# XinMing0411/AC-VAE

Measured on AMD Instinct MI355X. Metric: train-step captions/s (and audio-sec/s) at B=32, 1/2/4/8 MI355X, higher is better.
Workload: dtype f32

## Files before the change

acvae_amd/csrc/decoder.hip:

```cpp
#include <cstdlib>
#include <vector>
#include "common.h"
#include "conv.h"
#include "rnn.h"
#include "decode_persist.h"
#include "text_common.h"

namespace {

inline int gemm2(const float* A1, long lda1, const float* B1, long ldb1, int K1, const float* A2, long lda2,
                 const float* B2, long ldb2, int K2, const float* bias, float* C, long ldc, int M, int N, int acc,
                 const Ctx& st) {
  if (M <= 64)
    return acvae_gemm_nt_dual(A1, lda1, B1, ldb1, K1, A2, lda2, B2, ldb2, K2, bias, C, ldc, M, N, acc, st.s, st.skws);
  ACVAE_TRY(acvae_gemm_nt_dual(A1, lda1, B1, ldb1, K1, nullptr, 0, nullptr, 0, 0, bias, C, ldc, M, N, acc, st.s, st.skws));
  return acvae_gemm_nt_dual(A2, lda2, B2, ldb2, K2, nullptr, 0, nullptr, 0, 0, nullptr, C, ldc, M, N, 1, st.s, st.skws);
}
struct TnWs { float* p; long bytes; };
inline int gemm_tn(const float* A, long lda, const float* B, long ldb, float* C, long ldc, int M, int N, int K, TnWs ws,
                   hipStream_t st) {
  return acvae_gemm_tn_fused(A, lda, B, ldb, C, ldc, M, N, K, 0, ws.p, ws.bytes, st);
}
struct TnBatch {
  TnGroup g;
// ... 825 lines not shown
  int64_t* words_c = (int64_t*)(sc + L.words_c);
  ACVAE_TRY(acvae::gather_words(words, Tc, 1, words_c, N, Tc, st));
  ACVAE_TRY(fork.begin());

  float* d_out = sc + L.d_out;
  if (d_outputs_ext) ACVAE_TRY(acvae::copy_rows(d_out, H, d_outputs_ext, H, R, H, st));
  else ACVAE_TRY(zero(d_out, (long)R * H, st));
  if (d_p_means_utt) {
    float* dhid = sc + L.dhid;
    ACVAE_TRY(gemm(d_p_means_utt, 2 * E, wt_mlo, 2 * E, nullptr, dhid, H, N, H, 2 * E, 0, st));
    ACVAE_TRY(acvae::pool_bwd(dhid, lens1, (const int*)(sv + L.pool_arg), d_out, (long)Tc * H, H, 1, N, Tc, H, st));
  }
  if (d_logits) ACVAE_TRY(gemm(d_logits, V, wt_cls, V, nullptr, d_out, H, R, H, V, 1, st));
  auto heads_params = [&](const Ctx& c, TnWs ws, double* dp) -> int {
    acvae::ColsumBatch cb;
    if (d_p_means_utt) {
      ACVAE_TRY(gemm_tn(d_p_means_utt, 2 * E, sv + L.pool_hid, H, G(TP_MLO_W), H, 2 * E, H, N, ws, c));
      cb.add({d_p_means_utt, N, 2 * E, G(TP_MLO_B)});
    } else if (G(TP_MLO_W) && G(TP_MLO_B)) {
      ACVAE_TRY(zero(G(TP_MLO_W), (long)2 * E * H, c));
      ACVAE_TRY(zero(G(TP_MLO_B), 2 * E, c));
    }
    if (d_logits) {
      ACVAE_TRY(gemm_tn(d_logits, V, outputs, H, G(TP_DEC_CLS_W), H, V, H, R, ws, c));
      cb.add({d_logits, R, V, G(TP_DEC_CLS_B)});
    } else {
      ACVAE_TRY(zero(G(TP_DEC_CLS_W), (long)V * H, c));
      ACVAE_TRY(zero(G(TP_DEC_CLS_B), V, c));
    }
    return acvae::colsum_batch(cb, dp, L.dpart_doubles, c);
  };
  static const bool heads_aux = !(getenv("ACVAE_HEADS_AUX") && atoi(getenv("ACVAE_HEADS_AUX")) == 0);
  const bool heads_on_aux = heads_aux && fork.on();
  if (heads_on_aux) {
    ACVAE_TRY(heads_params(sp, tn_p, dpart_p));
  } else if (!defer) {
    ACVAE_TRY(heads_params(st, tn, dpart));
  }

  float* dgi = sc + L.dgi;
  float* dgh = sc + L.dgh;
  float* dqd = sc + L.dqd;
  float* dencproj = sc + L.dencproj;
  float* dvpart = sc + L.dvpart;
  float* dctx = sc + L.dctx;
  float* dmem = sc + L.dmem;
  float* dh = sc + L.dh_a;
  float* dh2 = sc + L.dh_b;
  const float* gru_save = sv + L.gru_save;
  const float* hprev_d = sv + L.hprev_d;
  const float* qd = sv + L.qd;
  auto dec_begin = [&]() -> int {
    ACVAE_TRY(zero(dencproj, (long)N * S * A, st));
    ACVAE_TRY(zero(dvpart, (long)N * A, st));
    ACVAE_TRY(zero(dmem, (long)N * S * E, st));
    ACVAE_TRY(zero(dh, (long)N * H, st));
    return ACVAE_OK;
  };
  float* drnn = sc + L.drnn;
  float* dz_dec = sc + L.dz_dec;
  int dv_rows = N;
  auto dec_bptt = [&](int t) -> int {
    ACVAE_TRY(acvae::gru_bwd(dh, H, d_out + (long)t * H, (long)Tc * H, gru_save + (long)t * 4 * H, (long)Tc * 4 * H,
                             hprev_d + (long)t * H, (long)Tc * H, dgi + (long)t * 3 * H, (long)Tc * 3 * H,
                             dgh + (long)t * 3 * H, (long)Tc * 3 * H, dh2, H, nullptr, t, N, H, st));
    ACVAE_TRY(gemm(dgi + (long)t * 3 * H, (long)Tc * 3 * H, wt_dih + (long)E * 3 * H, 3 * H, nullptr, dctx, E, N, E,
                   3 * H, 0, st));
    ACVAE_TRY(acvae_attn_bwd(dctx, E, 0, qd + (long)t * A, (long)Tc * A, A, sv + L.encproj_d, mem, mem_lens,
                             P(TP_DEC_ATT_V), attn_w + (long)t * S, (long)Tc * S, S, dqd + (long)t * A, (long)Tc * A, A,
                             dencproj, dmem, dvpart, sc + L.attws, L.attws_bytes, N, 1, S, A, E, st));
    ACVAE_TRY(gemm2(dgh + (long)t * 3 * H, (long)Tc * 3 * H, wt_dhh, 3 * H, 3 * H, dqd + (long)t * A, (long)Tc * A,
                    wt_datt, A, A, nullptr, dh2, H, N, H, 1, st));
    float* tmp = dh; dh = dh2; dh2 = tmp;
    return ACVAE_OK;
  };
  auto dec_memgrad = [&]() -> int {
    return gemm(dencproj, A, wt_datt + (long)H * A, A, nullptr, dmem, E, N * S, E, A, 1, st);
  };
  auto dec_dz = [&](const Ctx& c) -> int {
    ACVAE_TRY(gemm(dgi, 3 * H, wt_dih + (long)2 * E * 3 * H, 3 * H, nullptr, dz_dec, E, R, E, 3 * H, 0, c));
    if (!d_q_z) return ACVAE_OK;
    if (!prior_feeds_decoder) {
      ACVAE_TRY(acvae::copy_rows(d_q_z, E, dz_dec, E, R, E, c));
    } else {
      for (int t = 0; t < Tc; ++t)
        ACVAE_TRY(acvae::copy_rows(d_q_z + (long)t * E, (long)Tc * E, dis_flags_host[t] ? nullptr : dz_dec + (long)t * E,
                                   (long)Tc * E, N, E, c));
    }
    return ACVAE_OK;
  };
  auto dec_tn = [&](TnBatch& tb) -> int {
    ACVAE_TRY(tb.add(dgi, 3 * H, rnn_d, 3 * E, G(TP_DEC_WIH), 3 * E, 3 * H, 3 * E, R));
    ACVAE_TRY(tb.add(dgh, 3 * H, hprev_d, H, G(TP_DEC_WHH), H, 3 * H, H, R));
    ACVAE_TRY(tb.add(dqd, A, hprev_d, H, G(TP_DEC_ATT_W), E + H, A, H, R));
    return tb.add(dencproj, A, mem, E, G(TP_DEC_ATT_W) + H, E + H, A, E, N * S);
  };
  auto dec_params = [&](const Ctx& c, TnWs ws, double* dp, bool with_dz = true, bool with_tn = true) -> int {
    if (with_tn) {
      TnBatch tb{{}, ws, c};
      ACVAE_TRY(dec_tn(tb));
      ACVAE_TRY(tb.launch());
    }
    {
      acvae::ColsumBatch cb;
      cb.add({dgi, R, 3 * H, G(TP_DEC_BIH)}); cb.add({dgh, R, 3 * H, G(TP_DEC_BHH)});
      cb.add({dencproj, N * S, A, G(TP_DEC_ATT_B)}); cb.add({dvpart, dv_rows, A, G(TP_DEC_ATT_V)});
      ACVAE_TRY(acvae::colsum_batch(cb, dp, L.dpart_doubles, c));
    }
    ACVAE_TRY(gemm(dgi, 3 * H, wt_dih, 3 * H, nullptr, drnn, E, R, E, 3 * H, 0, c));
    if (emb_keep)
      ACVAE_TRY(acvae::dropout_rows(drnn, (long)Tc * E, E, emb_keep, E, (long)N * E, emb_drop_p < 1.f ? 1.f / (1.f - emb_drop_p) : 0.f, N, Tc, E, c));
    if (with_dz) ACVAE_TRY(dec_dz(c));
// ... 52 lines not shown
  float* dqp = sc + L.dqp;
  auto prior_memgrad = [&]() -> int {
    ACVAE_TRY(gemm(dgates, 4 * Hp, wt_pih, 4 * Hp, nullptr, drnn_p, 3 * E, R, 2 * E, 4 * Hp, 0, sp));
    ACVAE_TRY(zero(dencproj_p, (long)N * S * E, sp));
    ACVAE_TRY(zero(dvpart_p, (long)N * E, sp));
    ACVAE_TRY(acvae_attn_bwd(drnn_p + E, (long)Tc * 3 * E, 3 * E, sv + L.qp, (long)Tc * E, E, sv + L.encproj_p, mem,
                             mem_lens, P(TP_P_ATT_V), sv + L.attw_p, (long)Tc * S, S, dqp, (long)Tc * E, E, dencproj_p,
                             dmem_p, dvpart_p, sc + L.attws_p, L.attws_bytes, N, Tc, S, E, E, sp));
    return gemm(dencproj_p, E, wt_patt + (long)E * E, E, nullptr, dmem_p, E, N * S, E, E, 1, sp);
  };
  auto prior_tn_bptt = [&](TnBatch& tb) -> int {
    ACVAE_TRY(tb.add(dgates, 4 * Hp, rnn_p, 3 * E, G(TP_P_WIH), 3 * E, 4 * Hp, 3 * E, R));
    ACVAE_TRY(tb.add(dgates, 4 * Hp, hpprev, Hp, G(TP_P_WHH), Hp, 4 * Hp, Hp, R));
    return tb.add(dml_all, 2 * E, hp_all, Hp, G(TP_P_ML_W), Hp, 2 * E, Hp, R);
  };
  auto prior_params = [&](bool with_bptt_tn = true) -> int {
    {
      TnBatch tb{{}, tn_p, sp};
      if (with_bptt_tn) ACVAE_TRY(prior_tn_bptt(tb));
      ACVAE_TRY(tb.add(dqp, E, rnn_p, 3 * E, G(TP_P_ATT_W), 2 * E, E, E, R));
      ACVAE_TRY(tb.add(dencproj_p, E, mem, E, G(TP_P_ATT_W) + E, 2 * E, E, E, N * S));
      ACVAE_TRY(tb.launch());
    }
    {
      acvae::ColsumBatch cb;
      cb.add({dml_all, R, 2 * E, G(TP_P_ML_B)}); cb.add({dgates, R, 4 * Hp, G(TP_P_BIH), G(TP_P_BHH)});
      cb.add({dencproj_p, N * S, E, G(TP_P_ATT_B)}); cb.add({dvpart_p, N, E, G(TP_P_ATT_V)});
      ACVAE_TRY(acvae::colsum_batch(cb, dpart_p, L.dpart_doubles, sp));
    }
    ACVAE_TRY(gemm(dqp, E, wt_patt, E, nullptr, drnn_p, 3 * E, R, E, E, 1, sp));
    return acvae::embed_scatter(words_c, drnn_p, 3 * E, G(TP_P_EMB), V, R, E, sp);
  };
  bool early_tn = false;
  if (prior_feeds_decoder) {
    ACVAE_TRY(dec_begin());
    for (int t = Tc - 1; t >= 0; --t) ACVAE_TRY(dec_bptt(t));
    ACVAE_TRY(dec_memgrad());
    ACVAE_TRY(dec_params(st, tn, dpart));
    if (fork.on()) ACVAE_TRY(Fork::edge(st.s, sp.s));
    ACVAE_TRY(prior_begin());
    for (int t = Tc - 1; t >= 0; --t) ACVAE_TRY(prior_bptt(t));
    ACVAE_TRY(prior_memgrad());
    ACVAE_TRY(prior_params());
  } else if (persist_bwd) {
    PbParams pb{};
    pb.wt_dhh = wt_dhh; pb.wt_datt = wt_datt; pb.wt_dih = wt_dih; pb.wt_phh = wt_phh; pb.wt_pih = wt_pih; pb.wt_pml = wt_pml;
    pb.att_v = P(TP_DEC_ATT_V);
    pb.encproj = sv + L.encproj_d; pb.mem = mem; pb.qd = qd; pb.attn_w = attn_w; pb.gru_save = gru_save; pb.hprev_d = hprev_d;
    pb.lstm_save = lstm_save; pb.c_all = c_all; pb.p_logs = p_logs; pb.eps_p = eps_p; pb.mem_lens = mem_lens;
    pb.d_out = d_out; pb.d_p_z = d_p_z; pb.d_p_means = d_p_means; pb.d_p_logs = d_p_logs;
    pb.dgi = dgi; pb.dgh = dgh; pb.dqd = dqd; pb.dctx = drnn;
    pb.dencproj = dencproj; pb.dmem = dmem; pb.dvpart = dvpart; pb.dgates = dgates; pb.dml_all = dml_all; pb.dhp = dhp;
    pb.dctx_part = sc + L.pd_part; pb.dhp_part = pb.dctx_part + 4L * N * E; pb.dml_part = pb.dhp_part + 4L * N * E;
    pb.cnt = (unsigned*)(sc + L.pd_cnt_b);
    pb.dqd_part = sc + L.pd_dqd; pb.ctx = rnn_d + E;
    pb.N = N; pb.Tc = Tc; pb.S = S; pb.E = E; pb.H = H; pb.A = A;
    ACVAE_TRY(acvae::decode_persist_bwd(pb, st.s, flags));
    dv_rows = N * acvae::decode_persist_bwd_rc_splits(S);
    ACVAE_TRY(dec_memgrad());
    if (fork.on()) ACVAE_TRY(Fork::edge(st.s, sp.s));
    ACVAE_TRY(prior_memgrad());
    if (!defer) {
      ACVAE_TRY(dec_params(st, tn, dpart));
      ACVAE_TRY(prior_params());
    } else {
      TnBatch tb{{}, tn, st.s};
      ACVAE_TRY(dec_tn(tb));
      ACVAE_TRY(prior_tn_bptt(tb));
      ACVAE_TRY(tb.launch());
      early_tn = true;
    }
  } else {
    ACVAE_TRY(dec_begin());
    ACVAE_TRY(prior_begin());
    for (int t = Tc - 1; t >= 0; --t) {
      ACVAE_TRY(dec_bptt(t));
      ACVAE_TRY(prior_bptt(t));
    }
    ACVAE_TRY(dec_memgrad());
    ACVAE_TRY(prior_memgrad());
    if (!defer) {
      ACVAE_TRY(dec_params(st, tn, dpart));
      ACVAE_TRY(prior_params());
    }
  }
  ACVAE_TRY(fork.join());
  ACVAE_TRY(acvae::add_rows(dmem, E, dmem_p, E, N * S, E, st));
  if (has_ln) {
    ACVAE_TRY(transp(P(TP_LN_W), Eenc, wt_ln, E, E, Eenc, st));
    ACVAE_TRY(gemm(dmem, E, wt_ln, E, nullptr, d_mem_in, Eenc, N * S, Eenc, E, 0, st));
    ACVAE_TRY(gemm_tn(dmem, E, mem_in, Eenc, G(TP_LN_W), Eenc, E, Eenc, N * S, tn, st));
    ACVAE_TRY(acvae::colsum2(dmem, N * S, E, dpart, G(TP_LN_B), nullptr, 0, st));
  } else {
    ACVAE_TRY(acvae::copy_rows(d_mem_in, E, dmem, E, N * S, E, st));
  }
  if (defer) {
    ACVAE_TRY(dec_dz(st));
    ACVAE_TRY(Fork::edge(st.s, sp.s));
    if (!heads_on_aux) ACVAE_TRY(heads_params(sp, tn_p, dpart_p));
    ACVAE_TRY(dec_params(sp, tn_p, dpart_p, false, !early_tn));
    ACVAE_TRY(prior_params(!early_tn));
  }
  return ACVAE_OK;
}

extern "C" int acvae_caps_to_long(const float* caps, int64_t* out, int64_t n, void* stream) {
  if (!caps || !out || n <= 0) return ACVAE_EINVAL;
  return acvae::caps_to_long(caps, out, (long)n, (hipStream_t)stream);
}
```

acvae_amd/csrc/gemm.hip:

```cpp
#include <cstdint>
#include <cstdlib>
#include "mfma_tile.h"
#include "../../include/acvae_hip.h"
#include "conv.h"

namespace {
using namespace mfma;

template <int BN, bool VEC4>
__global__ __launch_bounds__(nt_threads<128>(), 2) void gemm_nt_kernel(const float* __restrict__ A, long lda,
                                                                     const float* __restrict__ B, long ldb,
                                                                     const float* __restrict__ bias,
                                                                     float* __restrict__ C, long ldc, int M, int N,
                                                                     int K, int accumulate) {
  __shared__ NtSmem<128, BN> sm;
  PlainLoader<VEC4, 4> al{A, lda, M, K};
  PlainLoader<VEC4, BN / 32> bl{B, ldb, N, K};
  PlainEpilogue ep{C, ldc, bias, accumulate};
  int bm, bn;
  xcd_tile(gridDim.x, gridDim.y, bm, bn);
  nt_block<128, BN>(al, bl, M, N, K, bm, bn, ep, sm);
}

template <int WM, int WN, bool VEC4>
__global__ __launch_bounds__(256, 2) void gemm_tn_kernel(const float* __restrict__ A, long lda,
                                                         const float* __restrict__ B, long ldb, float* __restrict__ C,
                                                         long ldc, int M, int N, int K, int k_per, int accumulate,
                                                         long slab_stride) {
  __shared__ TnSmem<WM, WN> sm;
  PlainKMajorLoader<VEC4> al{A, lda, M, K}, bl{B, ldb, N, K};
  const int kb = blockIdx.z * k_per;
  const int ke = min(K, kb + k_per);
// ... 134 lines not shown
        b[u] = q0 + u < S ? __hip_atomic_load(reinterpret_cast<const unsigned long long*>(base + (long)(q0 + u) * 1024 + e),
                                              __ATOMIC_RELAXED, __HIP_MEMORY_SCOPE_AGENT) : 0ull;
#pragma unroll
      for (int u = 0; u < 8; ++u)
        if (q0 + u < S) { v0 += __uint_as_float((unsigned)b[u]); v1 += __uint_as_float((unsigned)(b[u] >> 32)); }
    }
    const int mm = e >> 5, m = m0 + mm;
#pragma unroll
    for (int k = 0; k < 2; ++k) {
      const int n = n0 + (e & 31) + k;
      if (m < M && n < N) {
        float v = k ? v1 : v0;
        if (bias) v += bias[n];
        float* p = C + (long)m * ldc + n;
        if (accumulate) v += *p;
        *p = v;
      }
    }
    return;
  }
  for (int e = threadIdx.x; e < 1024; e += SK_THREADS) {
    const int mm = e >> 5, nn = e & 31;
    const int m = m0 + mm, n = n0 + nn;
    if (m < M && n < N) {
      float v = 0.f;
#pragma unroll
      for (int w = 0; w < SK_WAVES; ++w) v += red[w][mm][nn];
      if (bias) v += bias[n];
      float* p = C + (long)m * ldc + n;
      if (accumulate) v += *p;
      *p = v;
    }
  }
}

__global__ void transpose_kernel(const float* __restrict__ in, long ld_in, float* __restrict__ out, long ld_out,
                                 int rows, int cols) {
  __shared__ float tile[32][33];
  const int c0 = blockIdx.x * 32, r0 = blockIdx.y * 32;
  for (int j = threadIdx.y; j < 32; j += 8) {
    const int r = r0 + j, c = c0 + threadIdx.x;
    tile[j][threadIdx.x] = (r < rows && c < cols) ? in[(long)r * ld_in + c] : 0.f;
  }
  __syncthreads();
  for (int j = threadIdx.y; j < 32; j += 8) {
    const int c = c0 + j, r = r0 + threadIdx.x;
    if (r < rows && c < cols) out[(long)c * ld_out + r] = tile[threadIdx.x][j];
  }
}

__global__ void transpose_batch_kernel(TransposeBatch b) {
  __shared__ float tile[32][33];
  const int m = b.find((int)blockIdx.x);
  const TransposeJob& job = b.job[m];
  const int t = blockIdx.x - b.start[m];
  const int tcols = (job.cols + 31) / 32;
  const int c0 = (t % tcols) * 32, r0 = (t / tcols) * 32;
  const float* in = job.in;
  float* out = job.out;
  const int rows = job.rows, cols = job.cols;
  for (int j = threadIdx.y; j < 32; j += 8) {
    const int r = r0 + j, c = c0 + threadIdx.x;
    tile[j][threadIdx.x] = (r < rows && c < cols) ? in[(long)r * job.ld_in + c] : 0.f;
  }
  __syncthreads();
  for (int j = threadIdx.y; j < 32; j += 8) {
// ... 66 lines not shown

int acvae_gemm_nt_pair(const float* A0, int64_t lda0, const float* B0, int64_t ldb0, int K0, const float* bias0, float* C0,
                       int64_t ldc0, int N0, int acc0, const float* A1, int64_t lda1, const float* B1, int64_t ldb1, int K1,
                       const float* bias1, float* C1, int64_t ldc1, int N1, int acc1, int M, hipStream_t st) {
  if (!A0 || !B0 || !C0 || !A1 || !B1 || !C1 || M <= 0 || M > 64 || N0 <= 0 || N1 <= 0 || K0 <= 0 || K1 <= 0)
    return ACVAE_EINVAL;
  const bool vec = vec_ok(A0, lda0, K0) && vec_ok(B0, ldb0, K0) && vec_ok(A1, lda1, K1) && vec_ok(B1, ldb1, K1);
  const SkProblem p0{A0, lda0, B0, ldb0, K0, bias0, C0, ldc0, N0, acc0}, p1{A1, lda1, B1, ldb1, K1, bias1, C1, ldc1, N1, acc1};
  const int nx0 = cdiv(N0, 32);
  dim3 grid(nx0 + cdiv(N1, 32), cdiv(M, 32));
  if (vec) hipLaunchKernelGGL(gemm_skinny_pair_kernel<true>, grid, dim3(SK_THREADS), 0, st, p0, p1, nx0, M);
  else hipLaunchKernelGGL(gemm_skinny_pair_kernel<false>, grid, dim3(SK_THREADS), 0, st, p0, p1, nx0, M);
  ACVAE_LAUNCH_CHECK();
  return ACVAE_OK;
}

static int skinny_plan(int M, int N, int Ktot, bool dual, bool have_ws) {
  const long big_blocks = (long)cdiv(M, 128) * cdiv(N, N <= 64 ? 64 : 128);
  if (!(M <= 64 || dual || (big_blocks < 100 && M <= 4096))) return 0;
  const int tiles = cdiv(N, 32) * cdiv(M, 32);
  int S = 1;
  static const bool splitk_on = !(getenv("ACVAE_SKINNY_SPLITK") && getenv("ACVAE_SKINNY_SPLITK")[0] == '0');
  if (have_ws && splitk_on && tiles <= 16 && Ktot >= 1024) {
    S = 128 / tiles;
    const int maxs = Ktot / 256;
    if (S > maxs) S = maxs;
    if (S > 8) S = 8;
    if (S < 1) S = 1;
    if ((long)tiles * S > SK_MAX_TILES) S = 1;
  }
  return S;
}

int acvae_gemm_nt_dual(const float* A1, int64_t lda1, const float* B1, int64_t ldb1, int K1, const float* A2,
                       int64_t lda2, const float* B2, int64_t ldb2, int K2, const float* bias, float* C, int64_t ldc,
                       int M, int N, int accumulate, hipStream_t st, float* skws) {
  if (!A1 || !B1 || !C || M <= 0 || N <= 0 || K1 <= 0) return ACVAE_EINVAL;
  if (A2 && (!B2 || K2 <= 0)) return ACVAE_EINVAL;
  bool vec = vec_ok(A1, lda1, K1) && vec_ok(B1, ldb1, K1);
  if (A2) vec = vec && vec_ok(A2, lda2, K2) && vec_ok(B2, ldb2, K2);
  const int S = skinny_plan(M, N, K1 + (A2 ? K2 : 0), A2 != nullptr, skws != nullptr);
  if (S > 0) {
    dim3 grid(cdiv(N, 32), cdiv(M, 32), S);
    unsigned* cnt = (unsigned*)skws;
    float* slabs = skws ? skws + SK_MAX_TILES : nullptr;
    if (vec)
      hipLaunchKernelGGL(gemm_skinny_kernel<true>, grid, dim3(SK_THREADS), 0, st, A1, lda1, B1, ldb1, K1, A2, lda2, B2,
                         ldb2, K2, bias, C, ldc, M, N, accumulate, slabs, cnt);
    else
      hipLaunchKernelGGL(gemm_skinny_kernel<false>, grid, dim3(SK_THREADS), 0, st, A1, lda1, B1, ldb1, K1, A2, lda2,
                         B2, ldb2, K2, bias, C, ldc, M, N, accumulate, slabs, cnt);
    ACVAE_LAUNCH_CHECK();
    return ACVAE_OK;
  }
  const bool bn64 = (N <= 64);
  dim3 grid(cdiv(M, 128), cdiv(N, bn64 ? 64 : 128));
#define LAUNCH_NT(BN_, V_)                                                                                     \
  hipLaunchKernelGGL((gemm_nt_kernel<BN_, V_>), grid, dim3(nt_threads<128>()), 0, st, A1, lda1, B1, ldb1, bias, C, ldc, M, \
                     N, K1, accumulate)
  if (bn64) { if (vec) LAUNCH_NT(64, true); else LAUNCH_NT(64, false); }
  else      { if (vec) LAUNCH_NT(128, true); else LAUNCH_NT(128, false); }
#undef LAUNCH_NT
  ACVAE_LAUNCH_CHECK();
  return ACVAE_OK;
}

extern "C" int acvae_gemm_nt(const float* A, int64_t lda, const float* B, int64_t ldb, const float* bias, float* C,
                             int64_t ldc, int M, int N, int K, int accumulate, void* stream) {
  return acvae_gemm_nt_dual(A, lda, B, ldb, K, nullptr, 0, nullptr, 0, 0, bias, C, ldc, M, N, accumulate,
                            (hipStream_t)stream, nullptr);
}

static int tn_splits(int M, int N, int K) {
  const long tiles = (long)cdiv(M, 128) * cdiv(N, 128);
  int s = (int)(256 / (tiles > 0 ? tiles : 1));
// ... 100 lines not shown
      tk += j.gx * j.gy;
    }
  }
  if (tk > TN_TICKETS) return -1;
  g.seal([](const TnJob& j) { return j.gx * j.gy * j.slices; });
  return slab;
}

int acvae_gemm_tn_group(TnGroup& g, float* ws, int64_t ws_bytes, hipStream_t st) {
  if (!g.ok()) return ACVAE_EINVAL;
  if (g.n <= 0) return ACVAE_OK;
  const long slab = acvae_gemm_tn_group_plan(g);
  if (slab < 0 || (slab > 0 && (!ws || ws_bytes < ((int64_t)TN_TICKETS + slab) * (int64_t)sizeof(float)))) return ACVAE_EWORKSPACE;
  hipLaunchKernelGGL(gemm_tn_group_kernel, dim3(g.start[g.n]), dim3(256), 0, st, g, ws + TN_TICKETS,
                     reinterpret_cast<unsigned*>(ws));
  ACVAE_LAUNCH_CHECK();
  return ACVAE_OK;
}

extern "C" int acvae_transpose(const float* in, int64_t ld_in, float* out, int64_t ld_out, int rows, int cols,
                               void* stream) {
  if (!in || !out || rows <= 0 || cols <= 0) return ACVAE_EINVAL;
  hipLaunchKernelGGL(transpose_kernel, dim3(cdiv(cols, 32), cdiv(rows, 32)), dim3(32, 8), 0, (hipStream_t)stream, in,
                     ld_in, out, ld_out, rows, cols);
  ACVAE_LAUNCH_CHECK();
  return ACVAE_OK;
}

extern "C" int64_t acvae_gemm_nt_splitk_workspace_bytes(void) { return acvae_skinny_ws_floats() * (int64_t)sizeof(float); }
extern "C" int acvae_gemm_nt_split_plan(int M, int N, int K1, int K2, int with_ws) {
  if (M <= 0 || N <= 0 || K1 <= 0 || K2 < 0) return ACVAE_EINVAL;
  return skinny_plan(M, N, K1 + K2, K2 > 0, with_ws != 0);
}
extern "C" int acvae_gemm_nt_dual_ws(const float* A1, int64_t lda1, const float* B1, int64_t ldb1, int K1, const float* A2,
                                     int64_t lda2, const float* B2, int64_t ldb2, int K2, const float* bias, float* C,
                                     int64_t ldc, int M, int N, int accumulate, float* ws, int64_t ws_bytes, int reset_tickets,
                                     void* stream) {
  if (!A1 || !B1 || !C || M <= 0 || N <= 0 || K1 <= 0 || (A2 && (!B2 || K2 <= 0))) return ACVAE_EINVAL;
  if (ws && ws_bytes < acvae_gemm_nt_splitk_workspace_bytes()) return ACVAE_EWORKSPACE;
  hipStream_t st = (hipStream_t)stream;
  if (ws && reset_tickets) ACVAE_TRY(acvae_skinny_ws_reset(ws, st));
  return acvae_gemm_nt_dual(A1, lda1, B1, ldb1, K1, A2, lda2, B2, ldb2, K2, bias, C, ldc, M, N, accumulate, st, ws);
}
extern "C" int acvae_gemm_nt_pair_c(const float* A0, int64_t lda0, const float* B0, int64_t ldb0, int K0, const float* bias0,
                                    float* C0, int64_t ldc0, int N0, int acc0, const float* A1, int64_t lda1, const float* B1,
                                    int64_t ldb1, int K1, const float* bias1, float* C1, int64_t ldc1, int N1, int acc1, int M,
                                    void* stream) {
  return acvae_gemm_nt_pair(A0, lda0, B0, ldb0, K0, bias0, C0, ldc0, N0, acc0, A1, lda1, B1, ldb1, K1, bias1, C1, ldc1, N1,
                            acc1, M, (hipStream_t)stream);
}
extern "C" int64_t acvae_gemm_tn_fused_workspace_bytes(int M, int N, int K) {
  if (M <= 0 || N <= 0 || K <= 0) return -1;
  const int s = tn_splits(M, N, K);
  return s > 1 ? (int64_t)TN_TICKETS * 4 + (int64_t)s * M * N * (int64_t)sizeof(float) : 0;
}
extern "C" int acvae_gemm_tn_fused_plan(int M, int N, int K, int64_t ws_bytes) {
  if (M <= 0 || N <= 0 || K <= 0) return ACVAE_EINVAL;
  return tn_fused_slices(M, N, K, ws_bytes > 0, ws_bytes, nullptr);
}
extern "C" int acvae_gemm_tn_fused_c(const float* A, int64_t lda, const float* B, int64_t ldb, float* C, int64_t ldc, int M,
                                     int N, int K, int accumulate, float* ws, int64_t ws_bytes, int reset_tickets,
                                     void* stream) {
  if (!A || !B || !C || M <= 0 || N <= 0 || K <= 0) return ACVAE_EINVAL;
  hipStream_t st = (hipStream_t)stream;
  if (ws && reset_tickets && ws_bytes >= (int64_t)TN_TICKETS * 4)
    if (hipMemsetAsync(ws, 0, TN_TICKETS * sizeof(unsigned), st) != hipSuccess) return (int)hipGetLastError();
// ... 34 lines not shown
```

acvae_amd/csrc/mfma_tile.h:

```cpp
#pragma once
#include <type_traits>
#include "common.h"

namespace mfma {

constexpr int BK = 32;
constexpr int LDS_LD = BK + 4;
constexpr int KT = BK / 4;
constexpr int NT_LOADERS = 256;
constexpr int RPP = NT_LOADERS / KT;

template <int BMT, int BN>
struct alignas(16) NtSmem {
  alignas(16) float a[2][BMT * LDS_LD];
  alignas(16) float b[2][BN * LDS_LD];
};
template <int BMT>
constexpr int nt_threads() { return (BMT / 32 + 4) * 64; }

__device__ __forceinline__ void xcd_tile(int nm, int nn, int& bm, int& bn) {
#ifdef ACVAE_NO_XCD_REMAP
  bm = blockIdx.x; bn = blockIdx.y; return;
#endif
  const int total = nm * nn;
// ... 343 lines not shown
  constexpr int SK_U = 8;
  int g = wave;
  for (; g < Gfull; g += SK_U * nwaves) {
    float4 a[SK_U], b[SK_U];
#pragma unroll
    for (int u = 0; u < SK_U; ++u) {
      const int gu = g + u * nwaves;
      const long off = (gu < Gfull) ? (long)gu * 8 : 0;
      a[u] = *reinterpret_cast<const float4*>(ap + off);
      b[u] = *reinterpret_cast<const float4*>(bp + off);
    }
#pragma unroll
    for (int u = 0; u < SK_U; ++u) {
      const bool ok = (g + u * nwaves) < Gfull;
      const float4 av = ok ? a[u] : make_float4(0.f, 0.f, 0.f, 0.f);
      acc = __builtin_amdgcn_mfma_f32_32x32x2f32(av.x, b[u].x, acc, 0, 0, 0);
      acc = __builtin_amdgcn_mfma_f32_32x32x2f32(av.y, b[u].y, acc, 0, 0, 0);
      acc = __builtin_amdgcn_mfma_f32_32x32x2f32(av.z, b[u].z, acc, 0, 0, 0);
      acc = __builtin_amdgcn_mfma_f32_32x32x2f32(av.w, b[u].w, acc, 0, 0, 0);
    }
  }
  g = Gfull + ((wave - Gfull % nwaves) % nwaves + nwaves) % nwaves;
  for (; g < G; g += nwaves) {
    const int k = g * 8 + 4 * lh;
    const float4 a = sk_load<VEC4>(ap - 4 * lh, k, K);
    const float4 b = sk_load<VEC4>(bp - 4 * lh, k, K);
    acc = __builtin_amdgcn_mfma_f32_32x32x2f32(a.x, b.x, acc, 0, 0, 0);
    acc = __builtin_amdgcn_mfma_f32_32x32x2f32(a.y, b.y, acc, 0, 0, 0);
    acc = __builtin_amdgcn_mfma_f32_32x32x2f32(a.z, b.z, acc, 0, 0, 0);
    acc = __builtin_amdgcn_mfma_f32_32x32x2f32(a.w, b.w, acc, 0, 0, 0);
  }
}

}
```

acvae_amd/csrc/rnn.h:

```cpp
#pragma once
#include <hip/hip_runtime.h>
#include <stdint.h>
#include "job_table.h"
namespace acvae {
int caps_to_long(const float* caps, int64_t* out, long n, hipStream_t st);
int select_word(const int64_t* caps, long ld_caps, const int64_t* seqs, long ld_seqs, int64_t* words, long ld_words,
                int t, int use_caps, int start_idx, int N, hipStream_t st);
int finish_rows(int64_t* seqs, long ld_seqs, uint8_t* unfinished, int t, int end_idx, int N, hipStream_t st);
int embed_gather(const int64_t* words, long w_stride, const float* table, int V, float* out, long ld_out, int rows,
                 int E, hipStream_t st);
int embed_scatter(const int64_t* words_contig, const float* d, long ld_d, float* dtable, int V, int rows, int E,
                  hipStream_t st);
int dropout_rows(float* x, long ld_n, long ld_t, const uint8_t* keep, long k_sn, long k_st, float scale, int N, int cnt,
                 int E, hipStream_t st);
int gather_words(const int64_t* src, long s_sn, long s_st, int64_t* dst, int N, int T, hipStream_t st);
int gru_fwd(const float* gi, long ld_gi, const float* gh, long ld_gh, const float* hp, long ld_hp, float* ho,
            long ld_ho, float* oseq, long ld_os, float* save, long ld_sv, float* hps, long ld_hps, const int64_t* lens,
            int t, int N, int H, hipStream_t st);
int gru_bwd(const float* dh_next, long ld_dn, const float* d_out, long ld_do, const float* save, long ld_sv,
            const float* hps, long ld_hps, float* dgi, long ld_dgi, float* dgh, long ld_dgh, float* dh_prev, long ld_dp,
            const int64_t* lens, int t, int N, int H, hipStream_t st);
int lstm_fwd(const float* gates, long ld_g, const float* cp, long ld_cp, float* ho, long ld_ho, float* co, long ld_co,
             float* save, long ld_sv, int N, int H, hipStream_t st);
int lstm_bwd(const float* dh, long ld_dh, const float* dc_next, long ld_dc, const float* save, long ld_sv,
             const float* cp, long ld_cp, float* dgates, long ld_dg, float* dc_prev, long ld_dcp, int N, int H,
             hipStream_t st);
int pool_fwd(const float* x, long ld_n, long ld_t, const int64_t* lens, float* out, int* argmax, int N, int T, int C,
             hipStream_t st);
int pool_bwd(const float* d, const int64_t* lens, const int* argmax, float* dx, long ld_n, long ld_t, int accumulate,
             int N, int T, int C, hipStream_t st);
int colsum_rows(const float* x, long ld, int rows, int cols, float* out, int accumulate, hipStream_t st);
int add_rows(float* dst, long ld_d, const float* src, long ld_s, int rows, int cols, hipStream_t st);
int copy_rows(float* dst, long ld_d, const float* src, long ld_s, int rows, int cols, hipStream_t st);
struct CopyRowsJob { float* dst; long ld_d; const float* src; long ld_s; int rows, cols; };
using CopyRowsBatch = JobTable<CopyRowsJob, 8>;
int copy_rows_batch(const CopyRowsBatch& b, hipStream_t st);
struct ZeroRegion { void* p; long words; };
struct ZeroBatch : JobTable<ZeroRegion, 16> {
  void add(void* p, long words) { if (p && words > 0) JobTable::add({p, words}); }
};
int zero_batch(const ZeroBatch& b, hipStream_t st);
}
```

acvae_amd/csrc/rnn.hip:

```cpp
#include "common.h"
#include "rnn.h"

namespace {

constexpr int TH = 256;
inline int grid1(long n) {
  long b = (n + TH - 1) / TH;
  return (int)(b < 1 ? 1 : (b > 4096 ? 4096 : b));
}

__global__ void caps_to_long_kernel(const float* __restrict__ caps, int64_t* __restrict__ out, long n) {
  for (long i = blockIdx.x * (long)TH + threadIdx.x; i < n; i += (long)gridDim.x * TH) out[i] = (int64_t)caps[i];
}
__global__ void select_word_kernel(const int64_t* __restrict__ caps, long ld_caps, const int64_t* __restrict__ seqs,
                                   long ld_seqs, int64_t* __restrict__ words, long ld_words, int t, int use_caps,
                                   int start_idx, int N) {
  const int n = blockIdx.x * TH + threadIdx.x;
  if (n >= N) return;
  int64_t w;
  if (use_caps) w = caps[n * ld_caps + t];
  else if (t == 0) w = start_idx;
  else w = seqs[n * ld_seqs + t - 1];
  words[n * ld_words + t] = w;
}
// ... 190 lines not shown
                                int accumulate, int N, int T, int C) {
  const long total = (long)N * T * C;
  for (long i = blockIdx.x * (long)TH + threadIdx.x; i < total; i += (long)gridDim.x * TH) {
    const int c = (int)(i % C);
    const int t = (int)((i / C) % T);
    const int n = (int)(i / ((long)C * T));
    const int len = (int)lens[n];
    float g = 0.f;
    if (t < len) {
      const float dv = d[n * C + c];
      g = dv / (float)len + (argmax[n * C + c] == t ? dv : 0.f);
    }
    float* p = dx + n * ld_n + t * ld_t + c;
    *p = accumulate ? *p + g : g;
  }
}

__global__ void colsum_rows_kernel(const float* __restrict__ x, long ld, int rows, int cols, float* __restrict__ out,
                                   int accumulate) {
  const int c = blockIdx.x * TH + threadIdx.x;
  if (c >= cols) return;
  float a = 0.f;
  for (int r = 0; r < rows; ++r) a += x[r * ld + c];
  out[c] = accumulate ? out[c] + a : a;
}
__global__ void add_rows_kernel(float* __restrict__ dst, long ld_d, const float* __restrict__ src, long ld_s, int rows,
                                int cols) {
  const long total = (long)rows * cols;
  for (long i = blockIdx.x * (long)TH + threadIdx.x; i < total; i += (long)gridDim.x * TH) {
    const int r = (int)(i / cols), c = (int)(i % cols);
    dst[r * ld_d + c] += src[r * ld_s + c];
  }
}
__global__ void copy_rows_kernel(float* __restrict__ dst, long ld_d, const float* __restrict__ src, long ld_s, int rows,
                                 int cols) {
  const long total = (long)rows * cols;
  for (long i = blockIdx.x * (long)TH + threadIdx.x; i < total; i += (long)gridDim.x * TH) {
    const int r = (int)(i / cols), c = (int)(i % cols);
    dst[r * ld_d + c] = src ? src[r * ld_s + c] : 0.f;
  }
}

__global__ void copy_rows_batch_kernel(acvae::CopyRowsBatch b) {
  const acvae::CopyRowsJob& j = b.job[blockIdx.y];
  const long total = (long)j.rows * j.cols;
  for (long i = blockIdx.x * (long)TH + threadIdx.x; i < total; i += (long)gridDim.x * TH) {
    const int r = (int)(i / j.cols), c = (int)(i % j.cols);
    j.dst[r * j.ld_d + c] = j.src ? j.src[r * j.ld_s + c] : 0.f;
  }
}

__global__ void zero_batch_kernel(acvae::ZeroBatch b) {
  unsigned* p = static_cast<unsigned*>(b.job[blockIdx.y].p);
  const long n = b.job[blockIdx.y].words;
  for (long i = blockIdx.x * (long)TH + threadIdx.x; i < n; i += (long)gridDim.x * TH) p[i] = 0u;
}

}

namespace acvae {
#define LAUNCH(k, g, ...) hipLaunchKernelGGL(k, dim3(g), dim3(TH), 0, st, __VA_ARGS__)
int zero_batch(const ZeroBatch& b, hipStream_t st) {
  if (!b.ok()) return ACVAE_EINVAL;
  if (b.n <= 0) return ACVAE_OK;
  long most = 1;
  for (int j = 0; j < b.n; ++j) if (b.job[j].words > most) most = b.job[j].words;
// ... 61 lines not shown
         ld_dgh, dh_prev, ld_dp, lens, t, N, H);
  ACVAE_LAUNCH_CHECK(); return ACVAE_OK;
}
int lstm_fwd(const float* gates, long ld_g, const float* cp, long ld_cp, float* ho, long ld_ho, float* co, long ld_co,
             float* save, long ld_sv, int N, int H, hipStream_t st) {
  LAUNCH(lstm_fwd_kernel, grid1((long)N * H), gates, ld_g, cp, ld_cp, ho, ld_ho, co, ld_co, save, ld_sv, N, H);
  ACVAE_LAUNCH_CHECK(); return ACVAE_OK;
}
int lstm_bwd(const float* dh, long ld_dh, const float* dc_next, long ld_dc, const float* save, long ld_sv,
             const float* cp, long ld_cp, float* dgates, long ld_dg, float* dc_prev, long ld_dcp, int N, int H,
             hipStream_t st) {
  LAUNCH(lstm_bwd_kernel, grid1((long)N * H), dh, ld_dh, dc_next, ld_dc, save, ld_sv, cp, ld_cp, dgates, ld_dg, dc_prev,
         ld_dcp, N, H);
  ACVAE_LAUNCH_CHECK(); return ACVAE_OK;
}
int pool_fwd(const float* x, long ld_n, long ld_t, const int64_t* lens, float* out, int* argmax, int N, int T, int C,
             hipStream_t st) {
  LAUNCH(pool_fwd_kernel, grid1((long)N * C), x, ld_n, ld_t, lens, out, argmax, N, T, C);
  ACVAE_LAUNCH_CHECK(); return ACVAE_OK;
}
int pool_bwd(const float* d, const int64_t* lens, const int* argmax, float* dx, long ld_n, long ld_t, int accumulate,
             int N, int T, int C, hipStream_t st) {
  LAUNCH(pool_bwd_kernel, grid1((long)N * T * C), d, lens, argmax, dx, ld_n, ld_t, accumulate, N, T, C);
  ACVAE_LAUNCH_CHECK(); return ACVAE_OK;
}
int colsum_rows(const float* x, long ld, int rows, int cols, float* out, int accumulate, hipStream_t st) {
  LAUNCH(colsum_rows_kernel, cdiv(cols, TH), x, ld, rows, cols, out, accumulate);
  ACVAE_LAUNCH_CHECK(); return ACVAE_OK;
}
int add_rows(float* dst, long ld_d, const float* src, long ld_s, int rows, int cols, hipStream_t st) {
  LAUNCH(add_rows_kernel, grid1((long)rows * cols), dst, ld_d, src, ld_s, rows, cols);
  ACVAE_LAUNCH_CHECK(); return ACVAE_OK;
}
int copy_rows(float* dst, long ld_d, const float* src, long ld_s, int rows, int cols, hipStream_t st) {
  LAUNCH(copy_rows_kernel, grid1((long)rows * cols), dst, ld_d, src, ld_s, rows, cols);
  ACVAE_LAUNCH_CHECK(); return ACVAE_OK;
}
#undef LAUNCH
}
```

include/acvae_hip.h:

```cpp
#ifndef ACVAE_HIP_H
#define ACVAE_HIP_H
#include <stdint.h>
#ifdef __cplusplus
extern "C" {
#endif

#define ACVAE_ABI_VERSION 3
int acvae_abi_version(void);

#define ACVAE_FLAG_NO_PERSIST 1
#define ACVAE_FLAG_DEFER_PARAM_GRADS 2
#define ACVAE_FLAG_NO_ATTN_SPLIT 4
#define ACVAE_FLAG_ROLLOUT_GRAD 16
#define ACVAE_FLAG_TEST_STALL 8

int acvae_persist_status_register(int device, void* status_words_host);

int acvae_gemm_nt(const float* A, int64_t lda, const float* B, int64_t ldb, const float* bias, float* C,
                  int64_t ldc, int M, int N, int K, int accumulate, void* stream);
int acvae_gemm_tn(const float* A, int64_t lda, const float* B, int64_t ldb, float* C, int64_t ldc, int M, int N,
                  int K, int accumulate, float* slab_ws, int64_t slab_ws_bytes, void* stream);
int64_t acvae_gemm_tn_workspace_bytes(int M, int N, int K);
int64_t acvae_colsum_workspace_bytes(int cols);
int acvae_colsum(const float* x, int rows, int cols, float* out, void* ws, int64_t ws_bytes, void* stream);

int64_t acvae_gemm_nt_splitk_workspace_bytes(void);
int acvae_gemm_nt_split_plan(int M, int N, int K1, int K2, int with_ws);
int acvae_gemm_nt_dual_ws(const float* A1, int64_t lda1, const float* B1, int64_t ldb1, int K1, const float* A2,
                          int64_t lda2, const float* B2, int64_t ldb2, int K2, const float* bias, float* C, int64_t ldc,
                          int M, int N, int accumulate, float* ws, int64_t ws_bytes, int reset_tickets, void* stream);
int acvae_gemm_nt_pair_c(const float* A0, int64_t lda0, const float* B0, int64_t ldb0, int K0, const float* bias0, float* C0,
                         int64_t ldc0, int N0, int acc0, const float* A1, int64_t lda1, const float* B1, int64_t ldb1, int K1,
                         const float* bias1, float* C1, int64_t ldc1, int N1, int acc1, int M, void* stream);
int64_t acvae_gemm_tn_fused_workspace_bytes(int M, int N, int K);
int acvae_gemm_tn_fused_plan(int M, int N, int K, int64_t ws_bytes);
int acvae_gemm_tn_fused_c(const float* A, int64_t lda, const float* B, int64_t ldb, float* C, int64_t ldc, int M, int N,
                          int K, int accumulate, float* ws, int64_t ws_bytes, int reset_tickets, void* stream);
int64_t acvae_gemm_tn_group_workspace_bytes(int n, const int* M, const int* N, const int* K);
int acvae_gemm_tn_group_c(int n, const void* const* A, const int64_t* lda, const void* const* B, const int64_t* ldb,
                          const void* const* C, const int64_t* ldc, const int* M, const int* N, const int* K, void* ws,
                          int64_t ws_bytes, int reset_tickets, void* stream);
int64_t acvae_colsum_batch_workspace_bytes(int n, const int* P, const int* width);
int acvae_colsum_batch_plan(int n, const int* P, const int* width, int64_t ws_bytes);
int acvae_colsum_batch(int n, const void* const* x, const int* P, const int* width, const void* const* out,
                       const void* const* out_b, void* ws, int64_t ws_bytes, int reset_tickets, void* stream);
int acvae_transpose(const float* in, int64_t ld_in, float* out, int64_t ld_out, int rows, int cols, void* stream);

int64_t acvae_attn_fwd_workspace_bytes(int N, int Tq, int S, int A, int E);
int acvae_attn_fwd(const float* qproj, int64_t q_sn, int64_t q_sj, const float* encproj, const float* enc,
                   const int64_t* lens, const float* v, float* ctx, int64_t c_sn, int64_t c_sj, float* weights,
                   int64_t w_sn, int64_t w_sj, int N, int Tq, int S, int A, int E, void* ws, int64_t ws_bytes, void* stream,
                   int flags);
int acvae_tanh_att(const float* x, float* y, int64_t n, void* stream);
int64_t acvae_attn_bwd_workspace_bytes(int N, int Tq, int S, int A);
int acvae_attn_bwd(const float* dctx, int64_t dc_sn, int64_t dc_sj, const float* qproj, int64_t q_sn, int64_t q_sj,
                   const float* encproj, const float* enc, const int64_t* lens, const float* v,
                   const float* weights, int64_t w_sn, int64_t w_sj, float* dqproj, int64_t dq_sn, int64_t dq_sj,
                   float* dencproj, float* denc, float* dv_part, float* ws, int64_t ws_bytes, int N, int Tq, int S,
                   int A, int E, void* stream);

// ... 277 lines not shown
```

Measured before the change: 2116.

## Add register-blocked skinny GEMM, fuse backward glue copies, reorder heads fork

Result: no change. 2131 (median of 6 runs) (+0.7%).

```diff
diff --git a/acvae_amd/csrc/decoder.hip b/acvae_amd/csrc/decoder.hip
--- a/acvae_amd/csrc/decoder.hip
+++ b/acvae_amd/csrc/decoder.hip
@@ -881,7 +881,9 @@
   };
   static const bool heads_aux = !(getenv("ACVAE_HEADS_AUX") && atoi(getenv("ACVAE_HEADS_AUX")) == 0);
   const bool heads_on_aux = heads_aux && fork.on();
+  static const bool sw_heads_late = !(getenv("ACVAE_HEADS_LATE") && atoi(getenv("ACVAE_HEADS_LATE")) == 0);
   if (heads_on_aux) {
+    if (sw_heads_late) ACVAE_TRY(Fork::edge(st.s, sp.s));
     ACVAE_TRY(heads_params(sp, tn_p, dpart_p));
   } else if (!defer) {
     ACVAE_TRY(heads_params(st, tn, dpart));
@@ -926,7 +928,10 @@
   auto dec_memgrad = [&]() -> int {
     return gemm(dencproj, A, wt_datt + (long)H * A, A, nullptr, dmem, E, N * S, E, A, 1, st);
   };
+  static const bool sw_glue = !(getenv("ACVAE_BWD_GLUE") && atoi(getenv("ACVAE_BWD_GLUE")) == 0);
   auto dec_dz = [&](const Ctx& c) -> int {
+    if (sw_glue && d_q_z && !prior_feeds_decoder)
+      return gemm(dgi, 3 * H, wt_dih + (long)2 * E * 3 * H, 3 * H, nullptr, d_q_z, E, R, E, 3 * H, 0, c);
     ACVAE_TRY(gemm(dgi, 3 * H, wt_dih + (long)2 * E * 3 * H, 3 * H, nullptr, dz_dec, E, R, E, 3 * H, 0, c));
     if (!d_q_z) return ACVAE_OK;
     if (!prior_feeds_decoder) {
@@ -1045,6 +1050,7 @@
     return acvae::embed_scatter(words_c, drnn_p, 3 * E, G(TP_P_EMB), V, R, E, sp);
   };
   bool early_tn = false;
+  bool early_dz = false;
   if (prior_feeds_decoder) {
     ACVAE_TRY(dec_begin());
     for (int t = Tc - 1; t >= 0; --t) ACVAE_TRY(dec_bptt(t));
@@ -1077,6 +1083,7 @@
       ACVAE_TRY(dec_params(st, tn, dpart));
       ACVAE_TRY(prior_params());
     } else {
+      if (sw_glue) { ACVAE_TRY(dec_dz(st)); early_dz = true; }
       TnBatch tb{{}, tn, st.s};
       ACVAE_TRY(dec_tn(tb));
       ACVAE_TRY(prior_tn_bptt(tb));
@@ -1098,17 +1105,19 @@
     }
   }
   ACVAE_TRY(fork.join());
-  ACVAE_TRY(acvae::add_rows(dmem, E, dmem_p, E, N * S, E, st));
+  if (has_ln || !sw_glue) ACVAE_TRY(acvae::add_rows(dmem, E, dmem_p, E, N * S, E, st));
   if (has_ln) {
     ACVAE_TRY(transp(P(TP_LN_W), Eenc, wt_ln, E, E, Eenc, st));
     ACVAE_TRY(gemm(dmem, E, wt_ln, E, nullptr, d_mem_in, Eenc, N * S, Eenc, E, 0, st));
     ACVAE_TRY(gemm_tn(dmem, E, mem_in, Eenc, G(TP_LN_W), Eenc, E, Eenc, N * S, tn, st));
     ACVAE_TRY(acvae::colsum2(dmem, N * S, E, dpart, G(TP_LN_B), nullptr, 0, st));
+  } else if (sw_glue) {
+    ACVAE_TRY(acvae::sum_rows(d_mem_in, E, dmem, E, dmem_p, E, N * S, E, st));
   } else {
     ACVAE_TRY(acvae::copy_rows(d_mem_in, E, dmem, E, N * S, E, st));
   }
   if (defer) {
-    ACVAE_TRY(dec_dz(st));
+    if (!early_dz) ACVAE_TRY(dec_dz(st));
     ACVAE_TRY(Fork::edge(st.s, sp.s));
     if (!heads_on_aux) ACVAE_TRY(heads_params(sp, tn_p, dpart_p));
     ACVAE_TRY(dec_params(sp, tn_p, dpart_p, false, !early_tn));
diff --git a/acvae_amd/csrc/gemm.hip b/acvae_amd/csrc/gemm.hip
--- a/acvae_amd/csrc/gemm.hip
+++ b/acvae_amd/csrc/gemm.hip
@@ -1,3 +1,4 @@
+#include <atomic>
 #include <cstdint>
 #include <cstdlib>
 #include "mfma_tile.h"
@@ -198,6 +199,47 @@
       *p = v;
     }
   }
+}
+
+template <int BM, int BN, int U>
+__global__ __launch_bounds__(SK_THREADS) void gemm_skinny_blocked_kernel(const float* __restrict__ A, long lda,
+                                                                         const float* __restrict__ B, long ldb, int K,
+                                                                         const float* __restrict__ bias,
+                                                                         float* __restrict__ C, long ldc, int M, int N,
+                                                                         int accumulate) {
+  __shared__ float red[SK_WAVES][32][33];
+  const int lane = threadIdx.x & 63, wave = threadIdx.x >> 6, li = lane & 31, lh = lane >> 5;
+  const int n0 = blockIdx.x * (32 * BN), m0 = blockIdx.y * (32 * BM);
+  f32x16 acc[BM][BN];
+#pragma unroll
+  for (int i = 0; i < BM; ++i)
+#pragma unroll
+    for (int j = 0; j < BN; ++j)
+#pragma unroll
+      for (int r = 0; r < 16; ++r) acc[i][j][r] = 0.f;
+  sk_accumulate_blocked<BM, BN, U>(acc, A, lda, B, ldb, M, N, K, m0, n0, wave, li, lh);
+#pragma unroll
+  for (int i = 0; i < BM; ++i)
+#pragma unroll
+    for (int j = 0; j < BN; ++j) {
+      if (i | j) __syncthreads();
+#pragma unroll
+      for (int r = 0; r < 16; ++r) red[wave][(r & 3) + 8 * (r >> 2) + 4 * lh][li] = acc[i][j][r];
+      __syncthreads();
+      for (int e = threadIdx.x; e < 1024; e += SK_THREADS) {
+        const int mm = e >> 5, nn = e & 31;
+        const int m = m0 + 32 * i + mm, n = n0 + 32 * j + nn;
+        if (m < M && n < N) {
+          float v = 0.f;
+#pragma unroll
+          for (int w = 0; w < SK_WAVES; ++w) v += red[w][mm][nn];
+          if (bias) v += bias[n];
+          float* p = C + (long)m * ldc + n;
+          if (accumulate) v += *p;
+          *p = v;
+        }
+      }
+    }
 }
 
 __global__ void transpose_kernel(const float* __restrict__ in, long ld_in, float* __restrict__ out, long ld_out,
@@ -330,6 +372,58 @@
   return S;
 }
 
+static int device_cus() {
+  static std::atomic<int> cached[64];
+  int dev = 0;
+  if (hipGetDevice(&dev) != hipSuccess || dev < 0 || dev >= 64) { (void)hipGetLastError(); return 256; }
+  int n = cached[dev].load(std::memory_order_relaxed);
+  if (n == 0) {
+    if (hipDeviceGetAttribute(&n, hipDeviceAttributeMultiprocessorCount, dev) != hipSuccess || n <= 0) {
+      (void)hipGetLastError();
+      n = 256;
+    }
+    cached[dev].store(n, std::memory_order_relaxed);
+  }
+  return n;
+}
+static int skinny_block(int M, int N, int S, bool dual) {
+  static const bool on = !(getenv("ACVAE_SK_BLOCK") && atoi(getenv("ACVAE_SK_BLOCK")) == 0);
+  if (S != 1 || dual || !on) return 11;
+  const int tm = cdiv(M, 32), tn = cdiv(N, 32);
+  if ((long)tm * tn < device_cus()) return 11;
+  if (N > M) return tn >= 2 ? 12 : 11;
+  return tm >= 2 ? 21 : 11;
+}
+
+constexpr int SK_BLOCK_U = 4;
+template <int BM, int BN>
+static void launch_blocked(const float* A, int64_t lda, const float* B, int64_t ldb, int K, const float* bias, float* C,
+                           int64_t ldc, int M, int N, int accumulate, hipStream_t st) {
+  dim3 grid(cdiv(N, 32 * BN), cdiv(M, 32 * BM));
+  hipLaunchKernelGGL((gemm_skinny_blocked_kernel<BM, BN, SK_BLOCK_U>), grid, dim3(SK_THREADS), 0, st, A, lda, B, ldb, K, bias,
+                     C, ldc, M, N, accumulate);
+}
+static int skinny_launch(int block, const float* A, int64_t lda, const float* B, int64_t ldb, int K, const float* bias,
+                         float* C, int64_t ldc, int M, int N, int accumulate, hipStream_t st) {
+  switch (block) {
+    case 21: launch_blocked<2, 1>(A, lda, B, ldb, K, bias, C, ldc, M, N, accumulate, st); break;
+    case 12: launch_blocked<1, 2>(A, lda, B, ldb, K, bias, C, ldc, M, N, accumulate, st); break;
+    case 11: {
+      dim3 grid(cdiv(N, 32), cdiv(M, 32), 1);
+      if (vec_ok(A, lda, K) && vec_ok(B, ldb, K))
+        hipLaunchKernelGGL(gemm_skinny_kernel<true>, grid, dim3(SK_THREADS), 0, st, A, lda, B, ldb, K, nullptr, 0, nullptr, 0,
+                           0, bias, C, ldc, M, N, accumulate, nullptr, nullptr);
+      else
+        hipLaunchKernelGGL(gemm_skinny_kernel<false>, grid, dim3(SK_THREADS), 0, st, A, lda, B, ldb, K, nullptr, 0, nullptr, 0,
+                           0, bias, C, ldc, M, N, accumulate, nullptr, nullptr);
+      break;
+    }
+    default: return ACVAE_EINVAL;
+  }
+  ACVAE_LAUNCH_CHECK();
+  return ACVAE_OK;
+}
+
 int acvae_gemm_nt_dual(const float* A1, int64_t lda1, const float* B1, int64_t ldb1, int K1, const float* A2,
                        int64_t lda2, const float* B2, int64_t ldb2, int K2, const float* bias, float* C, int64_t ldc,
                        int M, int N, int accumulate, hipStream_t st, float* skws) {
@@ -339,6 +433,8 @@
   if (A2) vec = vec && vec_ok(A2, lda2, K2) && vec_ok(B2, ldb2, K2);
   const int S = skinny_plan(M, N, K1 + (A2 ? K2 : 0), A2 != nullptr, skws != nullptr);
   if (S > 0) {
+    const int block = vec ? skinny_block(M, N, S, A2 != nullptr) : 11;
+    if (block != 11) return skinny_launch(block, A1, lda1, B1, ldb1, K1, bias, C, ldc, M, N, accumulate, st);
     dim3 grid(cdiv(N, 32), cdiv(M, 32), S);
     unsigned* cnt = (unsigned*)skws;
     float* slabs = skws ? skws + SK_MAX_TILES : nullptr;
@@ -505,6 +601,18 @@
   if (M <= 0 || N <= 0 || K1 <= 0 || K2 < 0) return ACVAE_EINVAL;
   return skinny_plan(M, N, K1 + K2, K2 > 0, with_ws != 0);
 }
+extern "C" int acvae_gemm_nt_block_plan(int M, int N, int K1, int K2, int with_ws) {
+  if (M <= 0 || N <= 0 || K1 <= 0 || K2 < 0) return ACVAE_EINVAL;
+  const int S = skinny_plan(M, N, K1 + K2, K2 > 0, with_ws != 0);
+  return S > 0 ? skinny_block(M, N, S, K2 > 0) : 0;
+}
+extern "C" int acvae_gemm_nt_blocked_c(const float* A, int64_t lda, const float* B, int64_t ldb, const float* bias, float* C,
+                                       int64_t ldc, int M, int N, int K, int accumulate, int bm, int bn, void* stream) {
+  if (!A || !B || !C || M <= 0 || N <= 0 || K <= 0 || lda < K || ldb < K || ldc < N) return ACVAE_EINVAL;
+  if (bm < 1 || bn < 1 || bm * bn > 2) return ACVAE_EINVAL;
+  if (bm * bn > 1 && !(vec_ok(A, lda, K) && vec_ok(B, ldb, K))) return ACVAE_EALIGN;
+  return skinny_launch(bm * 10 + bn, A, lda, B, ldb, K, bias, C, ldc, M, N, accumulate, (hipStream_t)stream);
+}
 extern "C" int acvae_gemm_nt_dual_ws(const float* A1, int64_t lda1, const float* B1, int64_t ldb1, int K1, const float* A2,
                                      int64_t lda2, const float* B2, int64_t ldb2, int K2, const float* bias, float* C,
                                      int64_t ldc, int M, int N, int accumulate, float* ws, int64_t ws_bytes, int reset_tickets,
diff --git a/acvae_amd/csrc/mfma_tile.h b/acvae_amd/csrc/mfma_tile.h
--- a/acvae_amd/csrc/mfma_tile.h
+++ b/acvae_amd/csrc/mfma_tile.h
@@ -399,4 +399,54 @@
   }
 }
 
-}
+template <int BM, int BN, int U>
+__device__ __forceinline__ void sk_accumulate_blocked(f32x16 (&acc)[BM][BN], const float* A, long lda, const float* B,
+                                                      long ldb, int M, int N, int K, int m0, int n0, int wave, int li,
+                                                      int lh) {
+  const float* ap[BM];
+  const float* bp[BN];
+#pragma unroll
+  for (int i = 0; i < BM; ++i) ap[i] = A + (long)((m0 + 32 * i + li) < M ? m0 + 32 * i + li : 0) * lda + 4 * lh;
+#pragma unroll
+  for (int j = 0; j < BN; ++j) bp[j] = B + (long)((n0 + 32 * j + li) < N ? n0 + 32 * j + li : 0) * ldb + 4 * lh;
+  const int G = (K + 7) / 8, Gfull = K / 8;
+#define SK_BLOCK_MFMA(c_)                                                                              \
+  _Pragma("unroll") for (int i = 0; i < BM; ++i) _Pragma("unroll") for (int j = 0; j < BN; ++j)        \
+      acc[i][j] = __builtin_amdgcn_mfma_f32_32x32x2f32(av[i].c_, bv[j].c_, acc[i][j], 0, 0, 0)
+  int g = wave;
+  for (; g < Gfull; g += U * SK_WAVES) {
+    float4 a[U][BM], b[U][BN];
+#pragma unroll
+    for (int u = 0; u < U; ++u) {
+      const int gu = g + u * SK_WAVES;
+      const long off = (gu < Gfull) ? (long)gu * 8 : 0;
+#pragma unroll
+      for (int i = 0; i < BM; ++i) a[u][i] = *reinterpret_cast<const float4*>(ap[i] + off);
+#pragma unroll
+      for (int j = 0; j < BN; ++j) b[u][j] = *reinterpret_cast<const float4*>(bp[j] + off);
+    }
+#pragma unroll
+    for (int u = 0; u < U; ++u) {
+      const bool ok = (g + u * SK_WAVES) < Gfull;
+      float4 av[BM], bv[BN];
+#pragma unroll
+      for (int i = 0; i < BM; ++i) av[i] = ok ? a[u][i] : make_float4(0.f, 0.f, 0.f, 0.f);
+#pragma unroll
+      for (int j = 0; j < BN; ++j) bv[j] = b[u][j];
+      SK_BLOCK_MFMA(x); SK_BLOCK_MFMA(y); SK_BLOCK_MFMA(z); SK_BLOCK_MFMA(w);
+    }
+  }
+  g = Gfull + ((wave - Gfull % SK_WAVES) % SK_WAVES + SK_WAVES) % SK_WAVES;
+  for (; g < G; g += SK_WAVES) {
+    const int k = g * 8 + 4 * lh;
+    float4 av[BM], bv[BN];
+#pragma unroll
+    for (int i = 0; i < BM; ++i) av[i] = sk_load<true>(ap[i] - 4 * lh, k, K);
+#pragma unroll
+    for (int j = 0; j < BN; ++j) bv[j] = sk_load<true>(bp[j] - 4 * lh, k, K);
+    SK_BLOCK_MFMA(x); SK_BLOCK_MFMA(y); SK_BLOCK_MFMA(z); SK_BLOCK_MFMA(w);
+  }
+#undef SK_BLOCK_MFMA
+}
+
+}
diff --git a/acvae_amd/csrc/rnn.h b/acvae_amd/csrc/rnn.h
--- a/acvae_amd/csrc/rnn.h
+++ b/acvae_amd/csrc/rnn.h
@@ -31,6 +31,7 @@
              int N, int T, int C, hipStream_t st);
 int colsum_rows(const float* x, long ld, int rows, int cols, float* out, int accumulate, hipStream_t st);
 int add_rows(float* dst, long ld_d, const float* src, long ld_s, int rows, int cols, hipStream_t st);
+int sum_rows(float* dst, long ld_d, const float* a, long ld_a, const float* b, long ld_b, int rows, int cols, hipStream_t st);
 int copy_rows(float* dst, long ld_d, const float* src, long ld_s, int rows, int cols, hipStream_t st);
 struct CopyRowsJob { float* dst; long ld_d; const float* src; long ld_s; int rows, cols; };
 using CopyRowsBatch = JobTable<CopyRowsJob, 8>;
diff --git a/acvae_amd/csrc/rnn.hip b/acvae_amd/csrc/rnn.hip
--- a/acvae_amd/csrc/rnn.hip
+++ b/acvae_amd/csrc/rnn.hip
@@ -246,6 +246,14 @@
     dst[r * ld_d + c] += src[r * ld_s + c];
   }
 }
+__global__ void sum_rows_kernel(float* __restrict__ dst, long ld_d, const float* __restrict__ a, long ld_a,
+                                const float* __restrict__ b, long ld_b, int rows, int cols) {
+  const long total = (long)rows * cols;
+  for (long i = blockIdx.x * (long)TH + threadIdx.x; i < total; i += (long)gridDim.x * TH) {
+    const int r = (int)(i / cols), c = (int)(i % cols);
+    dst[r * ld_d + c] = a[r * ld_a + c] + b[r * ld_b + c];
+  }
+}
 __global__ void copy_rows_kernel(float* __restrict__ dst, long ld_d, const float* __restrict__ src, long ld_s, int rows,
                                  int cols) {
   const long total = (long)rows * cols;
@@ -373,6 +381,11 @@
   LAUNCH(add_rows_kernel, grid1((long)rows * cols), dst, ld_d, src, ld_s, rows, cols);
   ACVAE_LAUNCH_CHECK(); return ACVAE_OK;
 }
+int sum_rows(float* dst, long ld_d, const float* a, long ld_a, const float* b, long ld_b, int rows, int cols,
+             hipStream_t st) {
+  LAUNCH(sum_rows_kernel, grid1((long)rows * cols), dst, ld_d, a, ld_a, b, ld_b, rows, cols);
+  ACVAE_LAUNCH_CHECK(); return ACVAE_OK;
+}
 int copy_rows(float* dst, long ld_d, const float* src, long ld_s, int rows, int cols, hipStream_t st) {
   LAUNCH(copy_rows_kernel, grid1((long)rows * cols), dst, ld_d, src, ld_s, rows, cols);
   ACVAE_LAUNCH_CHECK(); return ACVAE_OK;
diff --git a/include/acvae_hip.h b/include/acvae_hip.h
--- a/include/acvae_hip.h
+++ b/include/acvae_hip.h
@@ -26,6 +26,9 @@
 
 int64_t acvae_gemm_nt_splitk_workspace_bytes(void);
 int acvae_gemm_nt_split_plan(int M, int N, int K1, int K2, int with_ws);
+int acvae_gemm_nt_block_plan(int M, int N, int K1, int K2, int with_ws);
+int acvae_gemm_nt_blocked_c(const float* A, int64_t lda, const float* B, int64_t ldb, const float* bias, float* C,
+                            int64_t ldc, int M, int N, int K, int accumulate, int bm, int bn, void* stream);
 int acvae_gemm_nt_dual_ws(const float* A1, int64_t lda1, const float* B1, int64_t ldb1, int K1, const float* A2,
                           int64_t lda2, const float* B2, int64_t ldb2, int K2, const float* bias, float* C, int64_t ldc,
                           int M, int N, int accumulate, float* ws, int64_t ws_bytes, int reset_tickets, void* stream);
```
